# kimwin2/ORB_SLAM2v2-1

Measured on AMD Instinct MI355X. Metric: frames/s ORB extract+match @1241x376 8-lvl 1000-feat, higher is better.
Workload: dtype u8; 1 GPU; kitti_stereo_1241x376_1000feat; frame=stereo pair (2 images), width=1241, height=376, nlevels=8, nfeatures=1000, ini_th_fast=20, min_th_fast=7, clock_ramp_steps=200, match=Frame::ComputeStereoMatches, parallelism=frames sharded over 1 GPU(s), world_size_observed=1, gauss_flavour=half_up

## Files before the change

### orb_slam2v2-1_amd/csrc/orbx_extract.hip

```cpp
#include "orbx_extract_dev.h"
#ifdef ORBX_DEVELOPER
#include "orbx_dev.h"
#endif
#include <math.h>
#include <float.h>
#include <stdarg.h>
#include <algorithm>

static thread_local char g_err[512] = "";
void orbx_set_error(const char *fmt, ...) {
    va_list ap;
    va_start(ap, fmt);
    vsnprintf(g_err, sizeof(g_err), fmt, ap);
    va_end(ap);
}
extern "C" const char *orbx_last_error(void) { return g_err; }
extern "C" const char *orbx_version(void) { return "orbx 0.1 (gfx950)"; }
extern "C" int orbx_device_count(void) {
    int n = 0;
    if (hipGetDeviceCount(&n) != hipSuccess) return 0;
    return n;
}

extern "C" int orbx_thread_release_scratch(void) {
// ... 309 lines not shown
    *bytes = need;
    return ORBX_OK;
}
static int launch_blur(orbx_extractor *h, const uint8_t *pyr, uint8_t **blurBuf, size_t *blurBytes, int b0, int B, hipStream_t st, unsigned *maskOut) {
    BlurPlan bp;
    int tiles = 0;
    const unsigned mask = blur_plan(h, bp, tiles);
    *maskOut = mask;
    if (!mask) return ORBX_OK;
    int rc = ensure_blur(h, blurBuf, blurBytes);
    if (rc) return rc;
    const size_t off = (size_t)b0 * h->sp.pyrImgBytes;
    hipLaunchKernelGGL(k_blur_levels, dim3((tiles + 3) / 4, B), dim3(256), 0, st, pyr + off, *blurBuf + off, h->sp.pyrImgBytes, h->d_geom, h->nlevels, tiles, bp,
                       h->flavour.gauss_rounding, gauss_taps_packed(h));
    return ORBX_OK;
}

static bool pyramid_fused_all(const orbx_extractor *h) { return h->opt[5] == 1 || h->scale_factor > 3.0; }
static void launch_pyramid(orbx_extractor *h, const uint8_t *d_imgs, uint8_t *pyr, int B, int stride, size_t img_stride, hipStream_t st) {
    const int nl = h->nlevels;
    if (pyramid_fused_all(h)) {
        hipLaunchKernelGGL(k_pyramid_fused, dim3(h->sp.pyrTilesX * h->sp.pyrTilesY, B), dim3(256), h->sp.pyrLdsBytes, st, d_imgs,
                           stride, img_stride, pyr, h->sp.pyrImgBytes, h->d_geom, nl, h->d_tab, h->sp.pyrXSpanOff,
                           h->sp.pyrYSpanOff, h->sp.pyrTilesX, h->sp.pyrTilesY, h->sp.pyrBufBytes, h->sp.pyrMaxPar, 0);
        return;
    }
    const bool hybrid = h->opt[5] == 3;
    const int lastSingle = hybrid ? std::min(2, nl - 1) : nl - 1;
    const LevelGeom &g0 = h->sp.geom[0];
    const size_t padLds = (size_t)PAD_ROWS_PER_BLOCK * stride + 32;
    if ((h->opt[24] == 2 || (h->opt[24] == 0 && B <= ORBX_HIST_IMAGES)) && padLds <= 60 * 1024)
        hipLaunchKernelGGL(k_pyr_pad_rows, dim3((g0.h + PAD_ROWS_PER_BLOCK - 1) / PAD_ROWS_PER_BLOCK, B), dim3(256), padLds, st, d_imgs, stride, img_stride, pyr,
                           h->sp.pyrImgBytes, h->d_geom);
    else
        hipLaunchKernelGGL(k_pyr_pad<true>, dim3(((g0.pstride >> 4) * g0.prows + 255) / 256, 1, B), dim3(256), 0, st, d_imgs, stride,
                           img_stride, pyr, h->sp.pyrImgBytes, h->d_geom, 0);
    const int cv = h->opt[25] == 3 ? 1 : 0;
    if (h->sp.nChains[cv] > 0 && !hybrid && (h->opt[5] == 4 || (h->opt[5] == 0 && h->opt[25] != 1 && B <= ORBX_HIST_IMAGES))) {
        for (int c = 0; c < h->sp.nChains[cv]; c++) {
            const ChainPlan &cp = h->sp.chains[cv][c];
            const size_t lds = 2 * (size_t)cp.bufBytes + (size_t)(cp.lb - cp.la) * cp.maxRows * 8;
            hipLaunchKernelGGL(k_pyr_chain, dim3(cp.tilesX * cp.tilesY, B), dim3(256), lds, st, pyr, h->sp.pyrImgBytes, h->d_geom, h->d_tab, cp);
        }
        return;
    }
    for (int l = 1; l <= lastSingle; l++) {
        const int nxc = (h->sp.geom[l].w + 1 + 127) / 128, nb16 = (h->sp.geom[l].h + 15) / 16, nb8 = (h->sp.geom[l].h + 7) / 8;
        const bool tall = h->scale_factor <= 1.25f && (h->opt[22] == 0 ? (size_t)nxc * nb16 * B >= 8192 : h->opt[22] == 2);
        if (tall)
            hipLaunchKernelGGL((k_pyr_level<16, 22>), dim3((nxc * nb16 + 3) / 4, B), dim3(256), 0, st, pyr, h->sp.pyrImgBytes, h->d_geom, l, h->d_tab, nxc, nb16);
        else
            hipLaunchKernelGGL((k_pyr_level<8, 12>), dim3((nxc * nb8 + 3) / 4, B), dim3(256), 0, st, pyr, h->sp.pyrImgBytes, h->d_geom, l, h->d_tab, nxc, nb8);
    }
    if (lastSingle < nl - 1)
        hipLaunchKernelGGL(k_pyramid_fused, dim3(h->sp.pyrTilesX * h->sp.pyrTilesY, B), dim3(256), h->sp.pyrLdsBytes, st, d_imgs,
                           stride, img_stride, pyr, h->sp.pyrImgBytes, h->d_geom, nl, h->d_tab, h->sp.pyrXSpanOff,
                           h->sp.pyrYSpanOff, h->sp.pyrTilesX, h->sp.pyrTilesY, h->sp.pyrBufBytes, h->sp.pyrMaxPar, lastSingle);
}

struct ChunkView {
    const uint8_t *imgs; uint8_t *pyr; uint32_t *cellCnt, *cellRaw, *slots, *cand, *lvlKp; uint16_t *nodeOf;
    int32_t *candCnt, *lvlCnt, *octFallback, *sparse; orbx_keypoint_t *kps; uint8_t *desc; int32_t *counts;
    int b0;
    size_t octSlot0;
};
static ChunkView chunk_view(const orbx_extractor *h, const uint8_t *d_imgs, size_t img_stride, orbx_keypoint_t *d_kps, uint8_t *d_desc,
                            int32_t *d_counts, int cap, int b0) {
    ChunkView v;
    const size_t z = (size_t)b0;
// ... 912 lines not shown
```

### orb_slam2v2-1_amd/csrc/orbx_extract_dev.h

```cpp
#pragma once
#include "orbx_internal.h"

__device__ __forceinline__ void wave_sync() {
    __builtin_amdgcn_fence(__ATOMIC_ACQ_REL, "workgroup");
    __builtin_amdgcn_wave_barrier();
}

__device__ __forceinline__ int wave_incl_scan_i32(int v) {
    v += __builtin_amdgcn_update_dpp(0, v, 0x111, 0xf, 0xf, true);
    v += __builtin_amdgcn_update_dpp(0, v, 0x112, 0xf, 0xf, true);
    v += __builtin_amdgcn_update_dpp(0, v, 0x114, 0xf, 0xf, true);
    v += __builtin_amdgcn_update_dpp(0, v, 0x118, 0xf, 0xf, true);
    v += __builtin_amdgcn_update_dpp(0, v, 0x142, 0xa, 0xf, true);
    v += __builtin_amdgcn_update_dpp(0, v, 0x143, 0xc, 0xf, true);
    return v;
}
__device__ __forceinline__ int wave_total_i32(int v) { return __builtin_amdgcn_readlane(wave_incl_scan_i32(v), 63); }

__device__ __forceinline__ int reflect101(int i, int n) {
    if (i < 0) i = -i;
    if (i >= n) i = 2 * (n - 1) - i;
    return i;
}
__device__ __forceinline__ int reflect101c(int p, int n) {
// ... 32 lines not shown
    int nb = 0;
    for (int l = 0; l < ORBX_MAX_LEVELS; l++) {
        blk0[l] = l <= lvBegin ? 0 : l < lvEnd ? nb : 0x7fffffff;
        if (l >= lvBegin && l < lvEnd) nb += (bound(l) + DESC_WAVES - 1) / DESC_WAVES;
    }
    return nb;
}
#define DESC_COPY_PER_BLOCK 16
#define BLUR_R 16
#define BLUR_SRC (BLUR_R + 6)
struct BlurPlan { int tileBase[ORBX_MAX_LEVELS + 1]; int tilesX[ORBX_MAX_LEVELS]; };
__global__ void k_blur_levels(const uint8_t *pyr, uint8_t *blur, size_t pyrImgBytes, const LevelGeom *geom, int nlevels, int totalTiles,
                              BlurPlan bp, int gaussRounding, uint32_t taps);
struct CellBases { int v[ORBX_MAX_LEVELS + 1]; };
__device__ __forceinline__ int level_of_cell(const CellBases &cb, int nlevels, int gc) {
    int l = 0;
#pragma unroll
    for (int i = 1; i < ORBX_MAX_LEVELS; i++) l += (i < nlevels && gc >= cb.v[i]) ? 1 : 0;
    return l;
}

__global__ void k_pyramid_fused(const uint8_t *src, int sstride, size_t simg, uint8_t *pyr, size_t pyrImgBytes, const LevelGeom *geom,
                                int nlevels, const int32_t *tab, int xSpanOff, int ySpanOff, int tilesX, int tilesY, int bufBytes,
                                int maxPar, int l0);
template <int RW, int SR>
__global__ void k_pyr_level(uint8_t *pyr, size_t pyrImgBytes, const LevelGeom *geom, int l, const int32_t *tab, int nxc,
                            int nbands);
template <bool FULL>
__global__ void k_pyr_pad(const uint8_t *img, int sstride, size_t simg, uint8_t *pyr, size_t pyrImgBytes, const LevelGeom *geom,
                          int l0);
__global__ void k_pyr_chain(uint8_t *pyr, size_t pyrImgBytes, const LevelGeom *geom, const int32_t *tab, ChainPlan cp);
__global__ void k_pyr_pad_rows(const uint8_t *img, int sstride, size_t simg, uint8_t *pyr, size_t pyrImgBytes, const LevelGeom *geom);
#define PAD_ROWS_PER_BLOCK 4
struct StripBases { int v[ORBX_MAX_LEVELS + 1]; };
__global__ void k_fast_strips(const uint8_t *pyr, size_t pyrImgBytes, const LevelGeom *geom, int nlevels, int totalStrips, int totalCells,
                              uint32_t *cellCnt, uint32_t *cellRaw, uint32_t *slots, size_t slotsPerImg, int iniTh, int minTh,
                              StripBases sb, const int32_t *sparseFlag, int strip0, int skipSparse);
__global__ void k_fast_strips_sparse(const uint8_t *pyr, size_t pyrImgBytes, const LevelGeom *geom, int nlevels, int totalStrips, int totalCells,
                                     uint32_t *cellCnt, uint32_t *cellRaw, uint32_t *slots, size_t slotsPerImg, int iniTh, int minTh,
                                     StripBases sb, const int32_t *sparseFlag);
struct FastHist { uint32_t *cnt, *best; int stride; const int32_t *tab; };
template <int ES_T, bool SPARSE>
__global__ void k_fast_cells(const uint8_t *pyr, size_t pyrImgBytes, const LevelGeom *geom, int nlevels, int totalCells,
                             uint32_t *cellCnt, uint32_t *cellRaw, uint32_t *slots, size_t slotsPerImg, int iniTh, int minTh, int ESrt,
                             int SSrt, int tileRows, int ldsPerWave, int phaseLimit, CellBases cb, unsigned stripLevels,
                             const int32_t *sparseFlag, FastHist fh);
__global__ void k_gather(const LevelGeom *geom, int nlevels, int totalCells, const uint32_t *cellCnt, const uint32_t *cellRaw,
                         const uint32_t *slots, size_t slotsPerImg, uint32_t *cand, size_t keysPerImg, int32_t *candCnt, int iniTh,
                         int minTh, CellBases cb, int32_t *sparseFlag, int sparsePerCell, int32_t *sparseSeen, int callSeq);
struct OctBig {
    uint32_t *part, *leaf, *best;
    int32_t *state;
    int K, nBig, deepMax, pyrMax;
    int levelOf[ORBX_MAX_LEVELS];
};
#define OCT_BIG_K 8
struct OctSrc {
    const uint32_t *cellCnt, *cellRaw, *slots;
    size_t slotsPerImg;
    int totalCells, iniTh, minTh;
    int32_t *candCntOut;
    int32_t *sparseFlag;
    int sparsePerCell;
    int32_t *sparseSeen;
    int callSeq;
    uint32_t *candOut;
// ... 33 lines not shown
```

### orb_slam2v2-1_amd/csrc/orbx_fast.hip

```cpp
#include "orbx_extract_dev.h"
#define FAST_STG 8
typedef short short2v __attribute__((ext_vector_type(2)));

typedef _Float16 half2v __attribute__((ext_vector_type(2)));
__device__ __forceinline__ half2v pk_min3(half2v a, half2v b, half2v c) {
    return __builtin_elementwise_minimum(__builtin_elementwise_minimum(a, b), c);
}
__device__ __forceinline__ half2v pk_max3(half2v a, half2v b, half2v c) {
    return __builtin_elementwise_maximum(__builtin_elementwise_maximum(a, b), c);
}

__device__ __forceinline__ half2v fast_ring_score(uint32_t vv, const uint32_t (&rr)[16]) {
    const half2v v = __builtin_bit_cast(half2v, vv);
    half2v d[16];
#pragma unroll
    for (int k = 0; k < 16; k++) d[k] = __builtin_bit_cast(half2v, rr[k]);
    half2v pmn[8], pmx[8];
#pragma unroll
    for (int t = 0; t < 8; t++) {
        pmn[t] = __builtin_elementwise_minimum(d[2 * t + 1], d[(2 * t + 2) & 15]);
        pmx[t] = __builtin_elementwise_maximum(d[2 * t + 1], d[(2 * t + 2) & 15]);
    }
    half2v qmn[8], qmx[8];
#pragma unroll
    for (int t = 0; t < 8; t++) {
        qmn[t] = __builtin_elementwise_minimum(pmn[t], pmn[(t + 1) & 7]);
        qmx[t] = __builtin_elementwise_maximum(pmx[t], pmx[(t + 1) & 7]);
    }
    half2v lo[8], hi[8];
#pragma unroll
    for (int t = 0; t < 8; t++) {
        const half2v e0 = d[2 * t], e1 = d[(2 * t + 9) & 15];
        lo[t] = pk_min3(qmn[t], qmn[(t + 2) & 7], __builtin_elementwise_maximum(e0, e1));
// ... 293 lines not shown
    if (strip >= totalStrips) return;
    int l = 0;
#pragma unroll
    for (int i = 1; i < ORBX_MAX_LEVELS; i++) l += (i < nlevels && strip >= sb.v[i]) ? 1 : 0;
    const LevelGeom g = geom[l];
    const bool pretest = sparseFlag != nullptr && __builtin_amdgcn_readfirstlane(sparseFlag[b * nlevels + l]) != 0;
    if (pretest && skipSparse) return;
    const int s = strip - sb.v[l];
    const int ng = (g.nCols + 3) >> 2;
    const int ci = s / ng, cj0 = 4 * (s - ci * ng);
    const int c = lane >> 4, j = lane & 15, cj = cj0 + c;
    const bool exists = cj < g.nCols;
    const int maxBX = g.w - ORBX_MINB, maxBY = g.h - ORBX_MINB;
    const int iniY = ORBX_MINB + ci * g.hCell, Xs = ORBX_MINB + cj0 * g.wCell;
    const int th = min(iniY + g.hCell + 6, maxBY) - iniY, ch = th - 6;
    const int cw = exists ? min(g.wCell, maxBX - (ORBX_MINB + cj * g.wCell) - 6) : 0;
    const int cw0 = min(g.wCell, maxBX - Xs - 6);
    const size_t cellIdx = (size_t)b * totalCells + g.cellBase + ci * g.nCols + cj;
    if (iniY >= maxBY - 3 || ch <= 0 || cw0 <= 0) {
        if (j == 0 && exists) { cellCnt[cellIdx] = 0; cellRaw[cellIdx] = 0; }
        return;
    }
    const int cjL = min(cj0 + 3, g.nCols - 1);
    const int tws = min(ORBX_MINB + cjL * g.wCell + g.wCell + 6, maxBX) - Xs;

    uint32_t *E = smem + wave * (STRIP_SLOTS * STRIP_ES);
    const size_t a = (size_t)(ORBX_EDGE + iniY) * g.pstride + ORBX_EDGE + Xs;
    const int sh = (int)(a & 3);
    const uint8_t *src = pyr + (size_t)b * pyrImgBytes + g.poff + (a - sh);
    const int nd = (sh + tws + 3) >> 2;
    const int qi = min(lane, nd - 1);
    const uint32_t loff = (uint32_t)qi * 4u;
    const int chS = __builtin_amdgcn_readfirstlane(ch), thS = __builtin_amdgcn_readfirstlane(th), pstrideS = __builtin_amdgcn_readfirstlane(g.pstride);
    auto load_row = [&](int r) -> uint2 {
        const uint32_t ro = (uint32_t)(min(r, thS - 1) * pstrideS);
        const uint32_t *p = (const uint32_t *)(src + ro + loff);
        uint2 d;
        d.x = p[0]; d.y = p[1];
        return d;
    };
    uint32_t *Ew = E + 4 * qi;
    auto write_row = [&](int slot, uint2 d) {
        uint4 e;
        e.x = __builtin_amdgcn_perm(d.y, d.x, 0x0c010c00u);
        e.y = __builtin_amdgcn_perm(d.y, d.x, 0x0c020c01u);
        e.z = __builtin_amdgcn_perm(d.y, d.x, 0x0c030c02u);
        e.w = __builtin_amdgcn_perm(d.y, d.x, 0x0c040c03u);
        *(uint4 *)(Ew + slot * STRIP_ES) = e;
    };
    {
        uint2 d[7];
#pragma unroll
        for (int r = 0; r < 7; r++) d[r] = load_row(r);
#pragma unroll
        for (int r = 0; r < 7; r++) write_row(r, d[r]);
    }
    uint2 pre = load_row(7);
    wave_sync();

    const int tlo = max(min(iniTh, minTh), 0), thi = max(iniTh, minTh);
    const int i0 = c * g.wCell + 3 + 2 * j;
    const uint32_t *q0 = E + sh + i0;
    const uint32_t vmask = (2 * j < cw ? 0xFFFFu : 0u) | (2 * j + 1 < cw ? 0xFFFF0000u : 0u);
    const uint32_t ltc = (1u << j) - 1u;
    const int cs = 16 * c;
    const half2v tl2 = __builtin_bit_cast(half2v, (uint32_t)tlo * 0x00010001u);
    const uint32_t x0 = (uint32_t)(cj * g.wCell + 3 + 2 * j), ybase = (uint32_t)(ci * g.hCell + 3);
    uint32_t *lvlSlots = slots + (size_t)b * slotsPerImg + g.slotOff;
    const uint32_t cellOff = (uint32_t)((ci * g.nCols + cj) * g.capc);
    uint32_t S1 = 0, H1 = 0, H2 = 0, LR1 = 0;
    uint32_t nRaw = 0, nHi = 0;
    auto rowstep = [&](const int R, int y, uint32_t &kpOut, uint32_t &sOut) {
        uint32_t S = 0;
        FPHASE("ring_reads");
        if (y < chS) {
            const uint32_t *q = q0;
#define SLOT(k) (((R + (k)) & 7) * STRIP_ES)
            const uint32_t vv = q[SLOT(3)];
            uint32_t rr[16];
            rr[0] = q[SLOT(6)];  rr[4] = q[SLOT(3) + 3];  rr[8] = q[SLOT(0)];  rr[12] = q[SLOT(3) - 3];
            bool go = true;
            FPHASE("row_pretest");
            if (pretest) {
                const half2v v = __builtin_bit_cast(half2v, vv), a0 = __builtin_bit_cast(half2v, rr[0]), a4 = __builtin_bit_cast(half2v, rr[4]),
                             a8 = __builtin_bit_cast(half2v, rr[8]), a12 = __builtin_bit_cast(half2v, rr[12]);
                const half2v ub = __builtin_elementwise_minimum(__builtin_elementwise_maximum(a0, a8), __builtin_elementwise_maximum(a4, a12)) - v;
                const half2v ud = v - __builtin_elementwise_maximum(__builtin_elementwise_minimum(a0, a8), __builtin_elementwise_minimum(a4, a12));
                const uint32_t u = __builtin_bit_cast(uint32_t, __builtin_elementwise_maximum(__builtin_elementwise_maximum(ub, ud), tl2) - tl2) & vmask;
                go = __ballot(u != 0) != 0;
            }
            FPHASE("ring_reads");
            if (go) {
                rr[1] = q[SLOT(6) + 1];   rr[2] = q[SLOT(5) + 2];   rr[3] = q[SLOT(4) + 3];
                rr[5] = q[SLOT(2) + 3];   rr[6] = q[SLOT(1) + 2];   rr[7] = q[SLOT(0) + 1];
                rr[9] = q[SLOT(0) - 1];   rr[10] = q[SLOT(1) - 2];  rr[11] = q[SLOT(2) - 3];
                rr[13] = q[SLOT(4) - 3];  rr[14] = q[SLOT(5) - 2];  rr[15] = q[SLOT(6) - 1];
                FPHASE("score");
                const half2v best = fast_ring_score(vv, rr);
                S = __builtin_bit_cast(uint32_t, __builtin_elementwise_maximum(best, (half2v){(_Float16)0, (_Float16)0})) & vmask;
            }
#undef SLOT
        }
        FPHASE("suppression");
        const uint32_t Lp = __builtin_amdgcn_perm(S, dpp_row_shr1(S), 0x05040302u);
        const uint32_t Rp = __builtin_amdgcn_perm(dpp_row_shl1(S), S, 0x05040302u);
        const half2v Lh = __builtin_bit_cast(half2v, Lp), Rh = __builtin_bit_cast(half2v, Rp), Sh = __builtin_bit_cast(half2v, S);
        const uint32_t H0 = __builtin_bit_cast(uint32_t, pk_max3(Lh, Sh, Rh));
        const uint32_t LR0 = __builtin_bit_cast(uint32_t, pk_max3(Lh, Rh, tl2));
        const half2v nb = pk_max3(__builtin_bit_cast(half2v, H2), __builtin_bit_cast(half2v, H0), __builtin_bit_cast(half2v, LR1));
        kpOut = __builtin_bit_cast(uint32_t, __builtin_bit_cast(half2v, S1) - nb);
        sOut = S1;
        S1 = S; H2 = H1; H1 = H0; LR1 = LR0;
        FPHASE("row_stream");
        if (y + 7 < thS) write_row((R + 7) & 7, pre);
        pre = load_row(y + 8);
        wave_sync();
    };
    auto rowpair = [&](const int R, int y) {
        uint32_t kpA, sA, kpB, sB;
        rowstep(R, y, kpA, sA);
        rowstep(R + 1, y + 1, kpB, sB);
        FPHASE("emission");
        const short2v fa = __builtin_bit_cast(short2v, kpA), fb = __builtin_bit_cast(short2v, kpB);
        const bool inA = fa.x > 0 || fa.y > 0, inB = fb.x > 0 || fb.y > 0;
        const unsigned long long mA = __ballot(inA), mB = __ballot(inB);
        if (mA | mB) {
            const uint32_t aA = (uint32_t)(mA >> cs) & 0xFFFFu, aB = (uint32_t)(mB >> cs) & 0xFFFFu;
            const bool second = inB ? fb.y > 0 : fa.y > 0;
            const uint32_t sv = inB ? sB : sA;
            const uint32_t sc = second ? sv >> 16 : sv & 0xFFFFu;
            const uint32_t pos = cellOff + nRaw + (inB ? __popc(aA) + __popc(aB & ltc) : __popc(aA & ltc));
            if (inA || inB)
                lvlSlots[pos] = (sc << 24) + (second ? x0 + 1u : x0) + ((ybase + (uint32_t)(y - 1) + (inB ? 1u : 0u)) << 12) - (1u << 24);
            nHi += (inA || inB) && sc > (uint32_t)thi ? 1u : 0u;
            nRaw += __popc(aA) + __popc(aB);
        }
    };
    FPHASE("loop");
    for (int yv = 0; yv <= chS; yv += 8) {
        const int y = __builtin_amdgcn_readfirstlane(yv);
        FPHASE("loop");
        rowpair(0, y);
        if (y + 2 <= chS) rowpair(2, y + 2);
        if (y + 4 <= chS) rowpair(4, y + 4);
        if (y + 6 <= chS) rowpair(6, y + 6);
    }
    FPHASE("epilogue");
#pragma unroll
    for (int o = 8; o > 0; o >>= 1) nHi += __shfl_xor(nHi, o);
    if (j == 0 && exists) {
        const uint32_t nA = iniTh >= minTh ? nHi : nRaw, nB = iniTh >= minTh ? nRaw : nHi;
        cellCnt[cellIdx] = min(nA ? nA : nB, (uint32_t)g.capc);
        cellRaw[cellIdx] = min(nRaw, (uint32_t)g.capc) | (nA ? 0x80000000u : 0u);
    }
}

#define SP_RS 144
#define SP_SLOTS 16
#define SP_MIRROR 6
#define SP_K 8
#define SP_LDS_PER_WAVE ((SP_SLOTS + SP_MIRROR) * SP_RS + SP_K * 64 * 2 + SP_K * 64 * 2 + 16)
__device__ __forceinline__ uint32_t lds_pair(const uint8_t *p) { return (uint32_t)p[0] | ((uint32_t)p[1] << 16); }

__global__ __launch_bounds__(64 * FAST_WAVES) __attribute__((amdgpu_waves_per_eu(7, 7))) void k_fast_strips_sparse(
    const uint8_t *__restrict__ pyr, size_t pyrImgBytes, const LevelGeom *__restrict__ geom, int nlevels, int totalStrips,
    int totalCells, uint32_t *__restrict__ cellCnt, uint32_t *__restrict__ cellRaw, uint32_t *__restrict__ slots, size_t slotsPerImg,
    int iniTh, int minTh, StripBases sb, const int32_t *__restrict__ sparseFlag) {
    __shared__ __align__(16) uint8_t smem[FAST_WAVES * SP_LDS_PER_WAVE];
    const int wave = __builtin_amdgcn_readfirstlane(threadIdx.x >> 6), lane = threadIdx.x & 63;
    int bx, b;
    xcd_block_map(bx, b);
    const int strip = bx * FAST_WAVES + wave;
    if (strip >= totalStrips) return;
    int l = 0;
#pragma unroll
    for (int i = 1; i < ORBX_MAX_LEVELS; i++) l += (i < nlevels && strip >= sb.v[i]) ? 1 : 0;
    if (__builtin_amdgcn_readfirstlane(sparseFlag[b * nlevels + l]) == 0) return;
    const LevelGeom g = geom[l];
    const int s = strip - sb.v[l];
    const int ng = (g.nCols + 3) >> 2;
    const int ci = s / ng, cj0 = 4 * (s - ci * ng);
    const int c = lane >> 4, j = lane & 15, cj = cj0 + c;
    const bool exists = cj < g.nCols;
// ... 239 lines not shown
```

### orb_slam2v2-1_amd/csrc/orbx_pyramid.hip

```cpp
#include "orbx_extract_dev.h"

__global__ __launch_bounds__(256) void k_pyramid_fused(
    const uint8_t *__restrict__ src, int sstride, size_t simg, uint8_t *__restrict__ pyr, size_t pyrImgBytes,
    const LevelGeom *__restrict__ geom, int nlevels, const int32_t *__restrict__ tab, int xSpanOff, int ySpanOff,
    int tilesX, int tilesY, int bufBytes, int maxPar, int l0) {
    extern __shared__ __align__(16) uint8_t smem[];
    uint2 *xpar = (uint2 *)(smem + 2 * bufBytes), *ypar = xpar + maxPar;
    __shared__ PyrSpan sX[ORBX_MAX_LEVELS], sY[ORBX_MAX_LEVELS];
    __shared__ int xo[ORBX_MAX_LEVELS + 1], yo[ORBX_MAX_LEVELS + 1];
    const int tid = threadIdx.x, tx = blockIdx.x % tilesX, ty = blockIdx.x / tilesX, b = blockIdx.y;
    if (tid < nlevels) sX[tid] = ((const PyrSpan *)(tab + xSpanOff))[tid * tilesX + tx];
    else if (tid >= 32 && tid < 32 + nlevels) sY[tid - 32] = ((const PyrSpan *)(tab + ySpanOff))[(tid - 32) * tilesY + ty];
    __syncthreads();
    if (tid == 0) {
        int ax = 0, ay = 0;
        for (int l = 0; l < nlevels; l++) {
            xo[l] = ax; yo[l] = ay;
            if (l > l0) { ax += sX[l].c1 - sX[l].c0; ay += sY[l].c1 - sY[l].c0; }
        }
        xo[nlevels] = ax; yo[nlevels] = ay;
    }
    __syncthreads();
    {
        const int nx = xo[nlevels], ny = yo[nlevels];
        for (int i = tid; i < nx + ny; i += 256) {
            const bool isx = i < nx;
            const int j = isx ? i : i - nx;
            const int *off = isx ? xo : yo;
            int l = l0 + 1;
            while (l + 1 <= nlevels && j >= off[l + 1]) l++;
            const LevelGeom *g = geom + l;
            const PyrSpan cs = isx ? sX[l] : sY[l], ps = isx ? sX[l - 1] : sY[l - 1];
            const int k = cs.c0 + (j - off[l]);
// ... 92 lines not shown
    const int wave = __builtin_amdgcn_readfirstlane(bx * 4 + (threadIdx.x >> 6)), lane = threadIdx.x & 63;
    if (wave >= nxc * nbands) return;
    const int band = wave / nxc, xc = wave - band * nxc;
    const LevelGeom G = geom[l];
    const int sw = geom[l - 1].w, sh = geom[l - 1].h, sps = geom[l - 1].pstride;
    uint8_t *base = pyr + (size_t)b * pyrImgBytes;
    const uint8_t *srow0 = base + geom[l - 1].poff + (size_t)ORBX_EDGE * sps;
    uint8_t *drow0 = base + G.poff + (size_t)ORBX_EDGE * G.pstride + ORBX_EDGE;
    const int x0 = xc * 128 + 2 * lane - 1, x1 = x0 + 1;
    const bool vst = x0 < G.w;
    const int xa = min(max(x0, 0), G.w - 1), xb = min(x1, G.w - 1);
    const int ca = ORBX_EDGE + tab[G.xofsOff + xa], cb = ORBX_EDGE + tab[G.xofsOff + xb];
    const uint32_t aa = (uint32_t)tab[G.xalphaOff + xa], ab = (uint32_t)tab[G.xalphaOff + xb];
    const int A = ca & ~3;
    const uint32_t oa = (uint32_t)(ca - A), ob = (uint32_t)(cb - A);
    const uint32_t selA = oa | ((oa + 1) << 16) | 0x0C000C00u, selB = ob | ((ob + 1) << 16) | 0x0C000C00u;
    (void)sw;
    const int y0 = band * RW, nrow = min(RW, G.h - y0);
    const int yl = min(y0 + (lane & RWM), G.h - 1);
    const int vsy = tab[G.yofsOff + yl];
    const uint32_t vbt = (uint32_t)tab[G.ybetaOff + yl];
    const int rf = __builtin_amdgcn_readfirstlane(vsy);
    const int kk = vsy + 1 - rf;
    const int prevsy = __shfl_up(vsy, 1);
    const bool okl = (lane & RWM) >= nrow || (rf >= 0 && vsy + 1 <= sh - 1 && kk < SR && ((lane & RWM) == 0 || vsy > prevsy));
    constexpr unsigned long long rowLanes = (1ull << RW) - 1ull;
    const bool regular = (__ballot(okl) & rowLanes) == rowLanes;
    if (regular) {
        uint32_t m = (lane & RWM) < nrow ? 1u << (kk & 31) : 0u;
        m |= __shfl_xor(m, 1); m |= __shfl_xor(m, 2); m |= __shfl_xor(m, 4);
        if (RW == 16) m |= __shfl_xor(m, 8);
        const uint32_t mask = __builtin_amdgcn_readfirstlane(m);
        const int lastk = 31 - __builtin_clz(mask | 1u);
        uint2 q[SR];
#pragma unroll
        for (int k = 0; k < SR; k++) {
            const uint8_t *rowp = srow0 + (uint32_t)(min(rf + k, sh - 1) * sps);
            q[k] = make_uint2(0u, 0u);
            if (k <= lastk) q[k] = *(const uint2 *)(rowp + (uint32_t)A);
        }
        uint32_t tpa = 0, tpb = 0;
        int cnt = 0;
        uint8_t *drow = drow0 + (size_t)y0 * G.pstride - 1;
        const uint32_t xoff = (uint32_t)(x0 + 1);
#pragma unroll
        for (int k = 0; k < SR; k++) {
            if (k > lastk) continue;
            const uint32_t tca = udot2_u16(__builtin_amdgcn_perm(q[k].y, q[k].x, selA), aa) & 0x7FFF0u;
            const uint32_t tcb = udot2_u16(__builtin_amdgcn_perm(q[k].y, q[k].x, selB), ab) & 0x7FFF0u;
            if (k > 0 && ((mask >> k) & 1u)) {
                const uint32_t bb = (uint32_t)__builtin_amdgcn_readlane((int)vbt, cnt);
                const uint32_t b0 = (bb & 0xFFFu) << 12, b1 = ((bb >> 16) & 0xFFFu) << 12;
                const uint32_t pa = (vmulhi24(b0, tpa) + vmulhi24(b1, tca) + 2) >> 2;
                const uint32_t pb = (vmulhi24(b0, tpb) + vmulhi24(b1, tcb) + 2) >> 2;
                if (vst) *(uint16_t *)(drow + xoff) = (uint16_t)(pa | (pb << 8));
                drow += G.pstride;
                cnt++;
            }
            tpa = tca; tpb = tcb;
        }
        return;
    }
    int cr0 = -1, cr1 = -1;
    uint32_t t0a = 0, t0b = 0, t1a = 0, t1b = 0;
    for (int y = y0; y < y0 + nrow; y++) {
        const int syy = tab[G.yofsOff + y];
        const uint32_t bb = (uint32_t)tab[G.ybetaOff + y];
        const int r0 = min(max(syy, 0), sh - 1), r1 = min(max(syy + 1, 0), sh - 1);
        if (r0 == cr1) { t0a = t1a; t0b = t1b; cr0 = cr1; }
        else if (r0 != cr0) {
            const uint2 q = *(const uint2 *)(srow0 + (size_t)r0 * sps + A);
            t0a = udot2_u16(__builtin_amdgcn_perm(q.y, q.x, selA), aa) & 0x7FFF0u;
            t0b = udot2_u16(__builtin_amdgcn_perm(q.y, q.x, selB), ab) & 0x7FFF0u;
            cr0 = r0;
        }
        if (r1 != cr1) {
            if (r1 == cr0) { t1a = t0a; t1b = t0b; }
            else {
                const uint2 q = *(const uint2 *)(srow0 + (size_t)r1 * sps + A);
                t1a = udot2_u16(__builtin_amdgcn_perm(q.y, q.x, selA), aa) & 0x7FFF0u;
                t1b = udot2_u16(__builtin_amdgcn_perm(q.y, q.x, selB), ab) & 0x7FFF0u;
            }
            cr1 = r1;
        }
        const uint32_t b0 = (bb & 0xFFFu) << 12, b1 = ((bb >> 16) & 0xFFFu) << 12;
        const uint32_t pa = (vmulhi24(b0, t0a) + vmulhi24(b1, t1a) + 2) >> 2;
        const uint32_t pb = (vmulhi24(b0, t0b) + vmulhi24(b1, t1b) + 2) >> 2;
        if (vst) *(uint16_t *)(drow0 + (size_t)y * G.pstride + x0) = (uint16_t)(pa | (pb << 8));
    }
}

template <bool FULL>
__global__ __launch_bounds__(256) void k_pyr_pad(const uint8_t *__restrict__ img, int sstride, size_t simg,
                                                 uint8_t *__restrict__ pyr, size_t pyrImgBytes,
                                                 const LevelGeom *__restrict__ geom, int l0) {
    const int l = l0 + blockIdx.y;
    const LevelGeom G = geom[l];
    uint8_t *lvl = pyr + (size_t)blockIdx.z * pyrImgBytes + G.poff;
    const uint8_t *src = FULL ? img + (size_t)blockIdx.z * simg : lvl + (size_t)ORBX_EDGE * G.pstride + ORBX_EDGE;
    const int ss = FULL ? sstride : G.pstride;
    const int pw4 = (G.w + 2 * ORBX_EDGE + 3) >> 2, rows = G.h + 2 * ORBX_EDGE;
    const int LW = (ORBX_EDGE >> 2) + 1, R0 = (ORBX_EDGE + G.w) >> 2, side = LW + (pw4 - R0);
    if (FULL) {
        const int pc = G.pstride >> 4, totalc = pc * rows;
        const int cI0 = (ORBX_EDGE + 15) >> 4, cI1 = max((G.w + ORBX_EDGE) >> 4, cI0);
        const int nI = cI1 - cI0, nE = pc - nI, totalI = nI * rows;
        for (int i = blockIdx.x * 256 + threadIdx.x; i < totalc; i += gridDim.x * 256) {
            int py, c;
            if (i < totalI) {
                py = i / nI;
                c = cI0 + (i - py * nI);
            } else {
                const int j = i - totalI;
                py = j / nE;
                const int k = j - py * nE;
                c = k < cI0 ? k : cI1 + (k - cI0);
            }
            const uint8_t *srow = src + (size_t)reflect101c(py - ORBX_EDGE, G.h) * ss;
            const int px = c * 16 - ORBX_EDGE;
            uint4 v;
            if (px >= 0 && px + 15 < G.w) __builtin_memcpy(&v, srow + px, 16);
            else {
                uint32_t t[4];
#pragma unroll
                for (int u = 0; u < 4; u++)
                    t[u] = (uint32_t)srow[reflect101c(px + 4 * u, G.w)] | ((uint32_t)srow[reflect101c(px + 4 * u + 1, G.w)] << 8) |
                           ((uint32_t)srow[reflect101c(px + 4 * u + 2, G.w)] << 16) | ((uint32_t)srow[reflect101c(px + 4 * u + 3, G.w)] << 24);
                v = make_uint4(t[0], t[1], t[2], t[3]);
            }
            *(uint4 *)(lvl + (size_t)py * G.pstride + c * 16) = v;
        }
        return;
    }
    const int total = 2 * ORBX_EDGE * pw4 + G.h * side;
    const unsigned Mp = (1u << 24) / (unsigned)pw4 + 1u, Ms = (1u << 24) / (unsigned)side + 1u;
    for (int i = blockIdx.x * 256 + threadIdx.x; i < total; i += gridDim.x * 256) {
        int py, p4;
        if (i < 2 * ORBX_EDGE * pw4) {
            const int r = (int)(((unsigned long long)(unsigned)i * Mp) >> 24);
            p4 = i - r * pw4;
            py = r < ORBX_EDGE ? r : G.h + r;
        } else {
            const int j = i - 2 * ORBX_EDGE * pw4, r = (int)(((unsigned long long)(unsigned)j * Ms) >> 24), k = j - r * side;
            py = ORBX_EDGE + r;
            p4 = k < LW ? k : R0 + (k - LW);
        }
        const uint8_t *srow = src + (size_t)reflect101c(py - ORBX_EDGE, G.h) * ss;
        const int px = p4 * 4 - ORBX_EDGE;
        const uint32_t v = (uint32_t)srow[reflect101c(px, G.w)] | ((uint32_t)srow[reflect101c(px + 1, G.w)] << 8) |
                           ((uint32_t)srow[reflect101c(px + 2, G.w)] << 16) | ((uint32_t)srow[reflect101c(px + 3, G.w)] << 24);
        *(uint32_t *)(lvl + (size_t)py * G.pstride + p4 * 4) = v;
    }
}

#define PAD_ROWS PAD_ROWS_PER_BLOCK
__global__ __launch_bounds__(256) void k_pyr_pad_rows(const uint8_t *__restrict__ img, int sstride, size_t simg, uint8_t *__restrict__ pyr,
                                                      size_t pyrImgBytes, const LevelGeom *__restrict__ geom) {
    extern __shared__ __align__(16) uint8_t rows_lds[];
    const LevelGeom G = geom[0];
    const int tid = threadIdx.x, r0 = blockIdx.x * PAD_ROWS, nr = min(PAD_ROWS, G.h - r0);
    const uint8_t *src = img + (size_t)blockIdx.y * simg;
    uint8_t *lvl = pyr + (size_t)blockIdx.y * pyrImgBytes + G.poff;
    const uintptr_t p0 = (uintptr_t)(src + (size_t)r0 * sstride), p1 = p0 + (size_t)(nr - 1) * sstride + G.w;
    const uintptr_t a0 = p0 & ~(uintptr_t)15;
// ... 139 lines not shown
```

Measured before the change: 116,000 frames/s.

## Use buffer-resource loads/stores in FAST and pyramid kernels; restructure full-image pad kernel

Switches row loads and slot/pixel stores in the FAST cell kernel and the pyramid level kernel to AMD raw buffer intrinsics with scalar offsets, so the compiler does less per-lane 64-bit address arithmetic. FAST emission is simplified: scores are clamped to zero so nonzero tests replace signed short checks, and the two ballot masks are packed with a single perm so one popcount gives the slot offset. The full-image pad kernel is restructured into row-block interior copying, several rows per thread with no divides, plus a separate edge path, with a new launch geometry. The changes risk subtle issues through buffer range sizing, and the pad path only runs for large batches.

```diff
diff --git a/orb_slam2v2-1_amd/csrc/orbx_bufaddr.h b/orb_slam2v2-1_amd/csrc/orbx_bufaddr.h
--- /dev/null
+++ b/orb_slam2v2-1_amd/csrc/orbx_bufaddr.h
@@ -0,0 +1,19 @@
+#pragma once
+#include <stdint.h>
+
+typedef __amdgpu_buffer_rsrc_t orbx_buf_t;
+typedef uint32_t orbx_u32x2 __attribute__((ext_vector_type(2)));
+
+__device__ __forceinline__ orbx_buf_t buf_make(const void *base, uint32_t bytes) {
+    return __builtin_amdgcn_make_buffer_rsrc(const_cast<void *>(base), (short)0, (int)bytes, 0x00020000);
+}
+__device__ __forceinline__ uint2 buf_load_b64(orbx_buf_t r, uint32_t voff, uint32_t soff) {
+    const orbx_u32x2 v = __builtin_amdgcn_raw_buffer_load_b64(r, (int)voff, (int)soff, 0);
+    return make_uint2(v.x, v.y);
+}
+__device__ __forceinline__ void buf_store_b16(orbx_buf_t r, uint32_t voff, uint32_t soff, uint16_t v) {
+    __builtin_amdgcn_raw_buffer_store_b16(v, r, (int)voff, (int)soff, 0);
+}
+__device__ __forceinline__ void buf_store_b32(orbx_buf_t r, uint32_t voff, uint32_t soff, uint32_t v) {
+    __builtin_amdgcn_raw_buffer_store_b32(v, r, (int)voff, (int)soff, 0);
+}
diff --git a/orb_slam2v2-1_amd/csrc/orbx_extract.hip b/orb_slam2v2-1_amd/csrc/orbx_extract.hip
--- a/orb_slam2v2-1_amd/csrc/orbx_extract.hip
+++ b/orb_slam2v2-1_amd/csrc/orbx_extract.hip
@@ -365,9 +365,13 @@
     if ((h->opt[24] == 2 || (h->opt[24] == 0 && B <= ORBX_HIST_IMAGES)) && padLds <= 60 * 1024)
         hipLaunchKernelGGL(k_pyr_pad_rows, dim3((g0.h + PAD_ROWS_PER_BLOCK - 1) / PAD_ROWS_PER_BLOCK, B), dim3(256), padLds, st, d_imgs, stride, img_stride, pyr,
                            h->sp.pyrImgBytes, h->d_geom);
-    else
-        hipLaunchKernelGGL(k_pyr_pad<true>, dim3(((g0.pstride >> 4) * g0.prows + 255) / 256, 1, B), dim3(256), 0, st, d_imgs, stride,
-                           img_stride, pyr, h->sp.pyrImgBytes, h->d_geom, 0);
+    else {
+        const int pc = g0.pstride >> 4, cI0 = (ORBX_EDGE + 15) >> 4, cI1 = std::max((g0.w + ORBX_EDGE) >> 4, cI0), nI = cI1 - cI0, nE = pc - nI;
+        const int threads = std::min(256, std::max(64, (nI + 63) & ~63)), gx = std::max(1, (nI + threads - 1) / threads);
+        const int rowBlocks = (g0.prows + PAD_FULL_ROWS - 1) / PAD_FULL_ROWS, edgeRows = (nE * g0.prows + gx * threads - 1) / (gx * threads);
+        hipLaunchKernelGGL(k_pyr_pad<true>, dim3(gx, rowBlocks + edgeRows, B), dim3(threads), 0, st, d_imgs, stride, img_stride, pyr,
+                           h->sp.pyrImgBytes, h->d_geom, 0);
+    }
     const int cv = h->opt[25] == 3 ? 1 : 0;
     if (h->sp.nChains[cv] > 0 && !hybrid && (h->opt[5] == 4 || (h->opt[5] == 0 && h->opt[25] != 1 && B <= ORBX_HIST_IMAGES))) {
         for (int c = 0; c < h->sp.nChains[cv]; c++) {
diff --git a/orb_slam2v2-1_amd/csrc/orbx_extract_dev.h b/orb_slam2v2-1_amd/csrc/orbx_extract_dev.h
--- a/orb_slam2v2-1_amd/csrc/orbx_extract_dev.h
+++ b/orb_slam2v2-1_amd/csrc/orbx_extract_dev.h
@@ -88,6 +88,7 @@
 __global__ void k_pyr_chain(uint8_t *pyr, size_t pyrImgBytes, const LevelGeom *geom, const int32_t *tab, ChainPlan cp);
 __global__ void k_pyr_pad_rows(const uint8_t *img, int sstride, size_t simg, uint8_t *pyr, size_t pyrImgBytes, const LevelGeom *geom);
 #define PAD_ROWS_PER_BLOCK 4
+#define PAD_FULL_ROWS 4
 struct StripBases { int v[ORBX_MAX_LEVELS + 1]; };
 __global__ void k_fast_strips(const uint8_t *pyr, size_t pyrImgBytes, const LevelGeom *geom, int nlevels, int totalStrips, int totalCells,
                               uint32_t *cellCnt, uint32_t *cellRaw, uint32_t *slots, size_t slotsPerImg, int iniTh, int minTh,
diff --git a/orb_slam2v2-1_amd/csrc/orbx_fast.hip b/orb_slam2v2-1_amd/csrc/orbx_fast.hip
--- a/orb_slam2v2-1_amd/csrc/orbx_fast.hip
+++ b/orb_slam2v2-1_amd/csrc/orbx_fast.hip
@@ -1,4 +1,5 @@
 #include "orbx_extract_dev.h"
+#include "orbx_bufaddr.h"
 #define FAST_STG 8
 typedef short short2v __attribute__((ext_vector_type(2)));
 
@@ -358,12 +359,10 @@
     const int qi = min(lane, nd - 1);
     const uint32_t loff = (uint32_t)qi * 4u;
     const int chS = __builtin_amdgcn_readfirstlane(ch), thS = __builtin_amdgcn_readfirstlane(th), pstrideS = __builtin_amdgcn_readfirstlane(g.pstride);
+    const orbx_buf_t rowBuf = buf_make(src, (uint32_t)g.pstride * (uint32_t)g.prows - (uint32_t)(a - sh));
     auto load_row = [&](int r) -> uint2 {
         const uint32_t ro = (uint32_t)(min(r, thS - 1) * pstrideS);
-        const uint32_t *p = (const uint32_t *)(src + ro + loff);
-        uint2 d;
-        d.x = p[0]; d.y = p[1];
-        return d;
+        return buf_load_b64(rowBuf, loff, ro);
     };
     uint32_t *Ew = E + 4 * qi;
     auto write_row = [&](int slot, uint2 d) {
@@ -388,14 +387,15 @@
     const int i0 = c * g.wCell + 3 + 2 * j;
     const uint32_t *q0 = E + sh + i0;
     const uint32_t vmask = (2 * j < cw ? 0xFFFFu : 0u) | (2 * j + 1 < cw ? 0xFFFF0000u : 0u);
-    const uint32_t ltc = (1u << j) - 1u;
+    const uint32_t ltc = (1u << j) - 1u, ltcB = 0xFFFFu | (ltc << 16);
     const int cs = 16 * c;
     const half2v tl2 = __builtin_bit_cast(half2v, (uint32_t)tlo * 0x00010001u);
     const uint32_t x0 = (uint32_t)(cj * g.wCell + 3 + 2 * j), ybase = (uint32_t)(ci * g.hCell + 3);
-    uint32_t *lvlSlots = slots + (size_t)b * slotsPerImg + g.slotOff;
-    const uint32_t cellOff = (uint32_t)((ci * g.nCols + cj) * g.capc);
+    const orbx_buf_t slotBuf = buf_make(slots + (size_t)b * slotsPerImg + g.slotOff, (uint32_t)g.keyCap * 4u);
+    const uint32_t cellOff4 = (uint32_t)((ci * g.nCols + cj) * g.capc) * 4u;
+    uint32_t slot4 = cellOff4;
     uint32_t S1 = 0, H1 = 0, H2 = 0, LR1 = 0;
-    uint32_t nRaw = 0, nHi = 0;
+    uint32_t nHi = 0;
     auto rowstep = [&](const int R, int y, uint32_t &kpOut, uint32_t &sOut) {
         uint32_t S = 0;
         FPHASE("ring_reads");
@@ -434,7 +434,7 @@
         const uint32_t H0 = __builtin_bit_cast(uint32_t, pk_max3(Lh, Sh, Rh));
         const uint32_t LR0 = __builtin_bit_cast(uint32_t, pk_max3(Lh, Rh, tl2));
         const half2v nb = pk_max3(__builtin_bit_cast(half2v, H2), __builtin_bit_cast(half2v, H0), __builtin_bit_cast(half2v, LR1));
-        kpOut = __builtin_bit_cast(uint32_t, __builtin_bit_cast(half2v, S1) - nb);
+        kpOut = __builtin_bit_cast(uint32_t, __builtin_elementwise_maximum(__builtin_bit_cast(half2v, S1) - nb, (half2v){(_Float16)0, (_Float16)0}));
         sOut = S1;
         S1 = S; H2 = H1; H1 = H0; LR1 = LR0;
         FPHASE("row_stream");
@@ -447,19 +447,19 @@
         rowstep(R, y, kpA, sA);
         rowstep(R + 1, y + 1, kpB, sB);
         FPHASE("emission");
-        const short2v fa = __builtin_bit_cast(short2v, kpA), fb = __builtin_bit_cast(short2v, kpB);
-        const bool inA = fa.x > 0 || fa.y > 0, inB = fb.x > 0 || fb.y > 0;
-        const unsigned long long mA = __ballot(inA), mB = __ballot(inB);
+        const bool inB = kpB != 0u;
+        const unsigned long long mA = __ballot(kpA != 0u), mB = __ballot(inB);
         if (mA | mB) {
-            const uint32_t aA = (uint32_t)(mA >> cs) & 0xFFFFu, aB = (uint32_t)(mB >> cs) & 0xFFFFu;
-            const bool second = inB ? fb.y > 0 : fa.y > 0;
+            const uint32_t T = __builtin_amdgcn_perm((uint32_t)(mB >> cs), (uint32_t)(mA >> cs), 0x05040100u);
+            const uint32_t k = kpA | kpB;
+            const bool second = k > 0xFFFFu;
             const uint32_t sv = inB ? sB : sA;
             const uint32_t sc = second ? sv >> 16 : sv & 0xFFFFu;
-            const uint32_t pos = cellOff + nRaw + (inB ? __popc(aA) + __popc(aB & ltc) : __popc(aA & ltc));
-            if (inA || inB)
-                lvlSlots[pos] = (sc << 24) + (second ? x0 + 1u : x0) + ((ybase + (uint32_t)(y - 1) + (inB ? 1u : 0u)) << 12) - (1u << 24);
-            nHi += (inA || inB) && sc > (uint32_t)thi ? 1u : 0u;
-            nRaw += __popc(aA) + __popc(aB);
+            const uint32_t pos4 = slot4 + 4u * __popc(T & (inB ? ltcB : ltc));
+            const uint32_t yrow = ((ybase + (uint32_t)(y - 1)) << 12) - (1u << 24);
+            if (k != 0u) buf_store_b32(slotBuf, pos4, 0u, (sc << 24) + (x0 + (second ? 1u : 0u)) + (inB ? yrow + (1u << 12) : yrow));
+            nHi += k != 0u && sc > (uint32_t)thi ? 1u : 0u;
+            slot4 += 4u * __popc(T);
         }
     };
     FPHASE("loop");
@@ -475,6 +475,7 @@
 #pragma unroll
     for (int o = 8; o > 0; o >>= 1) nHi += __shfl_xor(nHi, o);
     if (j == 0 && exists) {
+        const uint32_t nRaw = (slot4 - cellOff4) >> 2;
         const uint32_t nA = iniTh >= minTh ? nHi : nRaw, nB = iniTh >= minTh ? nRaw : nHi;
         cellCnt[cellIdx] = min(nA ? nA : nB, (uint32_t)g.capc);
         cellRaw[cellIdx] = min(nRaw, (uint32_t)g.capc) | (nA ? 0x80000000u : 0u);
diff --git a/orb_slam2v2-1_amd/csrc/orbx_pyramid.hip b/orb_slam2v2-1_amd/csrc/orbx_pyramid.hip
--- a/orb_slam2v2-1_amd/csrc/orbx_pyramid.hip
+++ b/orb_slam2v2-1_amd/csrc/orbx_pyramid.hip
@@ -1,4 +1,5 @@
 #include "orbx_extract_dev.h"
+#include "orbx_bufaddr.h"
 
 __global__ __launch_bounds__(256) void k_pyramid_fused(
     const uint8_t *__restrict__ src, int sstride, size_t simg, uint8_t *__restrict__ pyr, size_t pyrImgBytes,
@@ -157,16 +158,17 @@
         if (RW == 16) m |= __shfl_xor(m, 8);
         const uint32_t mask = __builtin_amdgcn_readfirstlane(m);
         const int lastk = 31 - __builtin_clz(mask | 1u);
+        const orbx_buf_t srcBuf = buf_make(srow0, (uint32_t)sps * (uint32_t)(geom[l - 1].prows - ORBX_EDGE));
+        const orbx_buf_t dstBuf = buf_make(base + G.poff, (uint32_t)G.pstride * (uint32_t)G.prows);
         uint2 q[SR];
 #pragma unroll
         for (int k = 0; k < SR; k++) {
-            const uint8_t *rowp = srow0 + (uint32_t)(min(rf + k, sh - 1) * sps);
-            q[k] = make_uint2(0u, 0u);
-            if (k <= lastk) q[k] = *(const uint2 *)(rowp + (uint32_t)A);
+            if (k > lastk) continue;
+            q[k] = buf_load_b64(srcBuf, (uint32_t)A, (uint32_t)(min(rf + k, sh - 1) * sps));
         }
         uint32_t tpa = 0, tpb = 0;
         int cnt = 0;
-        uint8_t *drow = drow0 + (size_t)y0 * G.pstride - 1;
+        uint32_t drow = (uint32_t)((ORBX_EDGE + y0) * G.pstride + ORBX_EDGE - 1);
         const uint32_t xoff = (uint32_t)(x0 + 1);
 #pragma unroll
         for (int k = 0; k < SR; k++) {
@@ -178,8 +180,8 @@
                 const uint32_t b0 = (bb & 0xFFFu) << 12, b1 = ((bb >> 16) & 0xFFFu) << 12;
                 const uint32_t pa = (vmulhi24(b0, tpa) + vmulhi24(b1, tca) + 2) >> 2;
                 const uint32_t pb = (vmulhi24(b0, tpb) + vmulhi24(b1, tcb) + 2) >> 2;
-                if (vst) *(uint16_t *)(drow + xoff) = (uint16_t)(pa | (pb << 8));
-                drow += G.pstride;
+                if (vst) buf_store_b16(dstBuf, xoff, drow, (uint16_t)(pa | (pb << 8)));
+                drow += (uint32_t)G.pstride;
                 cnt++;
             }
             tpa = tca; tpb = tcb;
@@ -219,7 +221,7 @@
 __global__ __launch_bounds__(256) void k_pyr_pad(const uint8_t *__restrict__ img, int sstride, size_t simg,
                                                  uint8_t *__restrict__ pyr, size_t pyrImgBytes,
                                                  const LevelGeom *__restrict__ geom, int l0) {
-    const int l = l0 + blockIdx.y;
+    const int l = FULL ? l0 : l0 + blockIdx.y;
     const LevelGeom G = geom[l];
     uint8_t *lvl = pyr + (size_t)blockIdx.z * pyrImgBytes + G.poff;
     const uint8_t *src = FULL ? img + (size_t)blockIdx.z * simg : lvl + (size_t)ORBX_EDGE * G.pstride + ORBX_EDGE;
@@ -227,34 +229,40 @@
     const int pw4 = (G.w + 2 * ORBX_EDGE + 3) >> 2, rows = G.h + 2 * ORBX_EDGE;
     const int LW = (ORBX_EDGE >> 2) + 1, R0 = (ORBX_EDGE + G.w) >> 2, side = LW + (pw4 - R0);
     if (FULL) {
-        const int pc = G.pstride >> 4, totalc = pc * rows;
+        const int pc = G.pstride >> 4;
         const int cI0 = (ORBX_EDGE + 15) >> 4, cI1 = max((G.w + ORBX_EDGE) >> 4, cI0);
-        const int nI = cI1 - cI0, nE = pc - nI, totalI = nI * rows;
-        for (int i = blockIdx.x * 256 + threadIdx.x; i < totalc; i += gridDim.x * 256) {
-            int py, c;
-            if (i < totalI) {
-                py = i / nI;
-                c = cI0 + (i - py * nI);
-            } else {
-                const int j = i - totalI;
-                py = j / nE;
-                const int k = j - py * nE;
-                c = k < cI0 ? k : cI1 + (k - cI0);
-            }
-            const uint8_t *srow = src + (size_t)reflect101c(py - ORBX_EDGE, G.h) * ss;
-            const int px = c * 16 - ORBX_EDGE;
-            uint4 v;
-            if (px >= 0 && px + 15 < G.w) __builtin_memcpy(&v, srow + px, 16);
-            else {
-                uint32_t t[4];
-#pragma unroll
-                for (int u = 0; u < 4; u++)
-                    t[u] = (uint32_t)srow[reflect101c(px + 4 * u, G.w)] | ((uint32_t)srow[reflect101c(px + 4 * u + 1, G.w)] << 8) |
-                           ((uint32_t)srow[reflect101c(px + 4 * u + 2, G.w)] << 16) | ((uint32_t)srow[reflect101c(px + 4 * u + 3, G.w)] << 24);
-                v = make_uint4(t[0], t[1], t[2], t[3]);
-            }
-            *(uint4 *)(lvl + (size_t)py * G.pstride + c * 16) = v;
-        }
+        const int nI = cI1 - cI0, nE = pc - nI;
+        const int rowBlocks = (rows + PAD_FULL_ROWS - 1) / PAD_FULL_ROWS;
+        if ((int)blockIdx.y < rowBlocks) {
+            const int i = blockIdx.x * blockDim.x + threadIdx.x;
+            if (i >= nI) return;
+            const uint32_t off = (uint32_t)i * 16u;
+            uint4 v[PAD_FULL_ROWS];
+#pragma unroll
+            for (int r = 0; r < PAD_FULL_ROWS; r++) {
+                const int py = min((int)blockIdx.y * PAD_FULL_ROWS + r, rows - 1);
+                const uint8_t *srow = src + (size_t)reflect101c(py - ORBX_EDGE, G.h) * ss + (cI0 * 16 - ORBX_EDGE);
+                __builtin_memcpy(&v[r], srow + off, 16);
+            }
+#pragma unroll
+            for (int r = 0; r < PAD_FULL_ROWS; r++) {
+                const int py = min((int)blockIdx.y * PAD_FULL_ROWS + r, rows - 1);
+                *(uint4 *)(lvl + (size_t)py * G.pstride + cI0 * 16 + off) = v[r];
+            }
+            return;
+        }
+        const int j = (((int)blockIdx.y - rowBlocks) * gridDim.x + blockIdx.x) * blockDim.x + threadIdx.x;
+        if (j >= nE * rows) return;
+        const int py = j / nE, k = j - py * nE;
+        const int c = k < cI0 ? k : cI1 + (k - cI0);
+        const uint8_t *srow = src + (size_t)reflect101c(py - ORBX_EDGE, G.h) * ss;
+        const int px = c * 16 - ORBX_EDGE;
+        uint32_t t[4];
+#pragma unroll
+        for (int u = 0; u < 4; u++)
+            t[u] = (uint32_t)srow[reflect101c(px + 4 * u, G.w)] | ((uint32_t)srow[reflect101c(px + 4 * u + 1, G.w)] << 8) |
+                   ((uint32_t)srow[reflect101c(px + 4 * u + 2, G.w)] << 16) | ((uint32_t)srow[reflect101c(px + 4 * u + 3, G.w)] << 24);
+        *(uint4 *)(lvl + (size_t)py * G.pstride + c * 16) = make_uint4(t[0], t[1], t[2], t[3]);
         return;
     }
     const int total = 2 * ORBX_EDGE * pw4 + G.h * side;
```

Result: faster. 119,800 frames/s (median of 6 runs) (+3.2%).
